# drowe67/pirip

Hardware: AMD Instinct MI355X
Metric: IQ Msamples/s demodulated (2-FSK Fs=240k Rs=10k); BER vs CPU ref (higher is better)
Workload: dtype f32

## Files before the change

pirip_amd/csrc/demod_simd.hpp:

```cpp
#pragma once
#include <hip/hip_runtime.h>

#include <cstdint>

#include "../../include/pirip_hip.h"

namespace pirip {

typedef float v2f __attribute__((ext_vector_type(2)));

__device__ __forceinline__ uint32_t fbits(float v) { return __builtin_bit_cast(uint32_t, v); }

__device__ __forceinline__ void wave_lds_sync()
{
    __builtin_amdgcn_fence(__ATOMIC_RELEASE, "wavefront");
    __builtin_amdgcn_wave_barrier();
    asm volatile("" ::: "memory");
    __builtin_amdgcn_fence(__ATOMIC_ACQUIRE, "wavefront");
}

#define PIRIP_DPP_F(old, src, ctrl, rmask) \
    __builtin_bit_cast(float, __builtin_amdgcn_update_dpp(__builtin_bit_cast(int, (float)(old)), __builtin_bit_cast(int, (float)(src)), ctrl, rmask, 0xf, false))

__device__ __forceinline__ float wave_sum(float v)
{
    v += PIRIP_DPP_F(0.f, v, 0x111, 0xf);
    v += PIRIP_DPP_F(0.f, v, 0x112, 0xf);
    v += PIRIP_DPP_F(0.f, v, 0x114, 0xf);
    v += PIRIP_DPP_F(0.f, v, 0x118, 0xf);
    v += PIRIP_DPP_F(0.f, v, 0x142, 0xa);
    v += PIRIP_DPP_F(0.f, v, 0x143, 0xc);
    return __builtin_bit_cast(float, __builtin_amdgcn_readlane(__builtin_bit_cast(int, v), 63));
}

#define PIRIP_DPP_REDUCE(op) \
        "s_nop 1\n\t" op " %0, %0, %0 row_shr:1 row_mask:0xf bank_mask:0xf\n\t" \
        "s_nop 1\n\t" op " %0, %0, %0 row_shr:2 row_mask:0xf bank_mask:0xf\n\t" \
        "s_nop 1\n\t" op " %0, %0, %0 row_shr:4 row_mask:0xf bank_mask:0xf\n\t" \
        "s_nop 1\n\t" op " %0, %0, %0 row_shr:8 row_mask:0xf bank_mask:0xf\n\t" \
        "s_nop 1\n\t" op " %0, %0, %0 row_bcast:15 row_mask:0xa bank_mask:0xf\n\t" \
        "s_nop 1\n\t" op " %0, %0, %0 row_bcast:31 row_mask:0xc bank_mask:0xf\n\t" \
        "s_nop 1\n\tv_readlane_b32 %1, %0, 63"

__device__ __forceinline__ void wave_argmax(float &v, int &idx)
{
    float red = v;
    int smax, smin;
    asm(PIRIP_DPP_REDUCE("v_max_f32_dpp") : "+v"(red), "=s"(smax));
    int cand = (__builtin_bit_cast(int, v) == smax) ? idx : 0x7fffffff;
    asm(PIRIP_DPP_REDUCE("v_min_i32_dpp") : "+v"(cand), "=s"(smin));
    v = __builtin_bit_cast(float, smax);
    idx = smin;
}

template <bool FINITE, bool NZ = false>
__device__ __forceinline__ float sqrt_rn_normal(float x)
{
    if (FINITE) {
        float q = __builtin_amdgcn_rsqf(x);
        if (!NZ) asm("v_min_f32 %0, %0, %1" : "+v"(q) : "v"(0x1p60f));
        const float y = x * q, h = 0.5f * q;
        return __builtin_fmaf(__builtin_fmaf(-y, y, x), h, y);
    }
    const float y = __builtin_amdgcn_sqrtf(x);
    const float ym = __builtin_bit_cast(float, __builtin_bit_cast(int, y) - 1);
    const float yp = __builtin_bit_cast(float, __builtin_bit_cast(int, y) + 1);
    const float rm = __builtin_fmaf(-ym, y, x);
    const float rp = __builtin_fmaf(-yp, y, x);
    float r = (rm <= 0.0f) ? ym : y;
    r = (rp > 0.0f) ? yp : r;
    return r;
}

__device__ __forceinline__ v2f cmul_x(v2f a, v2f t)
{
    v2f p2, r;
    asm("v_pk_mul_f32 %0, %2, %3 op_sel_hi:[0,1]\n\t"
        "v_pk_mul_f32 %1, %2, %3 op_sel:[1,1] op_sel_hi:[1,0]\n\t"
        "v_pk_add_f32 %0, %0, %1 neg_lo:[0,1]"
        : "=&v"(r), "=&v"(p2) : "v"(a), "v"(t));
    return r;
}
// ... 54 lines not shown
```

pirip_amd/csrc/fsk_demod_wave.hip:

```cpp
#include <hip/hip_runtime.h>

#include <cmath>
#include <cstdio>
#include <cstdlib>

#include "../../include/pirip_hip.h"
#include "demod_simd.hpp"
#include "fsk_device.hpp"

namespace pirip {

namespace {

constexpr int kWave = 64;

struct cf { float x, y; };

__device__ __forceinline__ float add_lane_up(float a, float b)
{
    float r;
    asm("v_add_f32_dpp %0, %1, %2 wave_shl:1 row_mask:0xf bank_mask:0xf bound_ctrl:0" : "=v"(r) : "v"(a), "v"(b));
    return r;
}

// ... 20 lines not shown
constexpr unsigned kQuickHi = 0x7c000000u;
__device__ __forceinline__ unsigned umin2(unsigned a, unsigned b) { return a < b ? a : b; }
__device__ __forceinline__ unsigned umin3(unsigned a, unsigned b, unsigned c)
{
    unsigned r;
    asm("v_min3_u32 %0, %1, %2, %3" : "=v"(r) : "v"(a), "v"(b), "v"(c));
    return r;
}

__device__ __forceinline__ v2f scale_lo(v2f h, v2f x)
{
    v2f r; asm("v_pk_mul_f32 %0, %1, %2 op_sel_hi:[0,1]" : "=v"(r) : "v"(h), "v"(x)); return r;
}
__device__ __forceinline__ v2f scale_hi(v2f h, v2f x)
{
    v2f r; asm("v_pk_mul_f32 %0, %1, %2 op_sel:[1,0] op_sel_hi:[1,1]" : "=v"(r) : "v"(h), "v"(x)); return r;
}
__device__ __forceinline__ float mag2(v2f w)
{
    v2f sq;
    asm("v_pk_mul_f32 %0, %1, %1" : "=v"(sq) : "v"(w));
    float r;
    asm("v_add_f32 %0, %1, %2" : "=v"(r) : "v"(sq.x), "v"(sq.y));
    return r;
}
__device__ __forceinline__ v2f smooth2(v2f sf, v2f mag, v2f k)
{
    v2f t;
    asm("v_pk_mul_f32 %0, %0, %3 op_sel_hi:[1,0]\n\t"
        "v_pk_mul_f32 %1, %2, %3 op_sel:[0,1] op_sel_hi:[1,1]\n\t"
        "v_pk_add_f32 %0, %0, %1"
        : "+v"(sf), "=&v"(t) : "v"(mag), "v"(k));
    return sf;
}

template <int FMT> struct InFmt;
template <> struct InFmt<PIRIP_IN_CU8_FSKDEMOD> { static constexpr int BPS = 2; static constexpr bool NEUTRAL_OK = true; static constexpr uint32_t NEUTRAL = 0x7F7F7F7Fu; };
template <> struct InFmt<PIRIP_IN_CU8_CSDR> { static constexpr int BPS = 2; static constexpr bool NEUTRAL_OK = false; static constexpr uint32_t NEUTRAL = 0x80808080u; };
template <> struct InFmt<PIRIP_IN_CS16> { static constexpr int BPS = 4; static constexpr bool NEUTRAL_OK = true; static constexpr uint32_t NEUTRAL = 0u; };
template <> struct InFmt<PIRIP_IN_CF32> { static constexpr int BPS = 8; static constexpr bool NEUTRAL_OK = true; static constexpr uint32_t NEUTRAL = 0u; };

__device__ __forceinline__ float cvt_s16(float x)
{
    const float hi = x * 0.00133514404296875f;
    return __builtin_fmaf(x, -0x1.e60f04p-20f, hi);
}
template <int FMT>
__device__ __forceinline__ v2f decode(const uint32_t *rw, int k)
{
    if (FMT == PIRIP_IN_CU8_FSKDEMOD || FMT == PIRIP_IN_CU8_CSDR) {
        const uint32_t v = rw[k >> 1];
        return cvt_u8_pair<FMT>(v2f{(k & 1) ? ubyte2(v) : ubyte0(v), (k & 1) ? ubyte3(v) : ubyte1(v)});
    } else if (FMT == PIRIP_IN_CS16) {
        const uint32_t v = rw[k];
        return v2f{cvt_s16((float)(short)(v & 0xffffu)), cvt_s16((float)((int)v >> 16))};
    } else {
        return v2f{__builtin_bit_cast(float, rw[2 * k]), __builtin_bit_cast(float, rw[2 * k + 1])};
    }
}
template <int FMT>
__device__ __forceinline__ v2f lds_sample(const unsigned char *p)
{
    if (FMT == PIRIP_IN_CU8_FSKDEMOD || FMT == PIRIP_IN_CU8_CSDR) {
        const uint32_t v = *(const uint16_t *)p;
        return cvt_u8_pair<FMT>(v2f{ubyte0(v), ubyte1(v)});
    } else if (FMT == PIRIP_IN_CS16) {
// ... 58 lines not shown
    static constexpr int NMEM = N + 2 * TS;
    static constexpr int Q = TS / 4;
    static constexpr int HIST = 2 * TS + Q;
    static constexpr int STEP = TS / P;
    static constexpr int NLANES = NSYM + 2;
    static constexpr int NFFT = (N - Q) / (NDFT / 2) - 1;
    static constexpr int GUARD_B = ((HIST * BPS + 15) / 16) * 16;
    static constexpr int SUP_B = (N + Q) * BPS;
    static constexpr int NDMA16 = SUP_B / 1024;
    static constexpr int NDMA4 = (SUP_B - NDMA16 * 1024 + 255) / 256;
    static constexpr bool DIRECT = FMT == PIRIP_IN_CF32 && NDFT >= 256;
    static constexpr int HEAD_B = 1024, DUMP_B = 256;
    static_assert(!DIRECT || ((TS + Q) * BPS <= HEAD_B && 3 * TS >= 2 * TS + Q), "the head holds blocks 0..2's new samples");
    static constexpr int RAW_B = DIRECT ? GUARD_B + HEAD_B + DUMP_B : GUARD_B + NDMA16 * 1024 + NDMA4 * 256;
    static constexpr int XPS256 = 16 * 17 * 8;
    static constexpr int XP_FFT_B = NDFT == 256 ? 4 * XPS256 : NDFT == 512 ? 4480 : 8 * 72 * 8;
    static constexpr int XP_B = cmax(cmax(XP_FFT_B, NDFT * 4), NDFT == 256 ? 64 * 20 * 4 : NDFT == 128 ? 8 * 136 * 4 : 0);
    static constexpr int TAIL_DW = HIST * BPS / 4;
    static constexpr int TRAILER_DW = GUARD_B / 4;
    static_assert((HIST * BPS) % 4 == 0 && (GUARD_B - HIST * BPS) % 4 == 0, "tail copies move whole dwords");
    static_assert(GUARD_B + (2 * M + 1) * 4 <= M * HIST * 8, "the state block holds the raw tail and its trailer");
    static constexpr int CHS = (BPS == 2) ? TS : (TS % 8 == 0 ? 8 : TS % 4 == 0 ? 4 : 2);
    static constexpr int CH_DW = CHS * BPS / 4;
    static_assert(TS % 2 == 0 && TS % P == 0 && P >= 4, "bad Ts / P");
    static_assert(NLANES <= kWave, "one lane per symbol block");
    static_assert((TS * BPS) % 16 == 0 && (CHS * BPS) % 16 == 0 && TS % CHS == 0, "block and chunk strides keep 16-byte alignment");
    static_assert((N + Q) / (NDFT / 2) - 1 == NFFT && N / (NDFT / 2) - 1 == NFFT, "numffts must not depend on nin");
    static_assert(NDFT == 256 ? (NFFT >= 4) : NDFT == 512 ? (NFFT % 2 == 0) : (NDFT == 128 && NFFT <= 8),
                  "FFT batches (Ndft = 256: the last batch of 4 may be partial; Ndft = 128: one batch of up to eight)");
    static_assert((NFFT - 1) * (NDFT / 2) + NDFT <= N - Q, "FFT windows stay inside the shortest frame");
    static_assert(M * P <= 48, "window prefix sums are kept in registers");
};

template <class C, int M> constexpr int wave_lds_bytes() { return C::RAW_B + C::XP_B; }

}

template <int M, int TS, int P, int NSYM, int NDFT, int FMT, int WPB, int WPS, bool FFT_FMA = false, bool MASK = false, int BAND = 0>
__global__ __launch_bounds__(kWave * WPB, WPS) void fsk_demod_wave_kernel(DemodArgs a_kernarg, int nstreams)
{
    constexpr bool INPLACE = TS == 10;
    static_assert(offsetof(DemodArgs, d) == 0, "the argument block is the first kernel argument");
    auto ap = [&]() {
        if constexpr (INPLACE) return (const __attribute__((address_space(4))) DemodArgs *)__builtin_amdgcn_kernarg_segment_ptr();
        else return (const DemodArgs *)&a_kernarg;
    }();
#define PIRIP_ARGS_REREAD() do { if constexpr (INPLACE) asm volatile("" : "+s"(ap)); } while (0)
#define a (*ap)
#define d (ap->d)
    static_assert(BAND == 0 || ((BAND == 2 || BAND == 4) && NDFT == 256 && !MASK), "band-only estimator: Ndft = 256, peak method, 32 or 64 bins");
    auto cmul = [](v2f x, v2f t) { return FFT_FMA ? rot_step(x, t) : cmul_x(x, t); };
    using C = WaveCfg<M, TS, P, NSYM, NDFT, FMT>;
    constexpr int N = C::N, NMEM = C::NMEM, HIST = C::HIST, STEP = C::STEP, Q = C::Q, BPS = C::BPS;
    constexpr int GUARD_B = C::GUARD_B;

    __shared__ __attribute__((aligned(16))) unsigned char s_raw[WPB][C::RAW_B];
    __shared__ __attribute__((aligned(16))) unsigned char s_xp[WPB][C::XP_B];
    constexpr int TAB_F = NDFT == 256 ? 12 * 16 * 4 : NDFT == 512 ? 8 * 16 * 2 + 12 * 32 * 2 : 8 * 16 * 2;
    __shared__ __attribute__((aligned(16))) float s_tab[TAB_F];
    __shared__ __attribute__((aligned(16))) float2 s_tph[P];
    __shared__ __attribute__((aligned(16))) float2 s_tgain[NSYM + 2];
    __shared__ float s_misc[WPB][3];
    extern __shared__ __attribute__((aligned(16))) float s_lnI0[];

    const int lane0 = threadIdx.x & (kWave - 1);
    const int wv = __builtin_amdgcn_readfirstlane(threadIdx.x >> 6);
    const int sid = blockIdx.x * WPB + wv;

    if (NDFT == 256) {
        for (int i = threadIdx.x; i < 12 * 16; i += kWave * WPB)
            ((float4 *)s_tab)[i] = ((const float4 *)a.t.fast_tab)[(i & 15) * 12 + (i >> 4)];
    } else {
        for (int i = threadIdx.x; i < TAB_F / 4; i += kWave * WPB) ((float4 *)s_tab)[i] = ((const float4 *)(a.t.fast_tab + NDFT))[i];
    }
    if constexpr (P <= 10) if (a.io.soft.llr) {
        if (a.io.soft.llr_map == kLlrRician) { for (int i = threadIdx.x; i < 258; i += kWave * WPB) s_lnI0[i] = a.io.soft.lnI0[i]; }
        else if (threadIdx.x < 20) {
            const int sg = threadIdx.x >> 2, cc = threadIdx.x & 3;
            const float c2 = sg == 0 ? 0.226f : sg == 1 ? 0.1245f : sg == 2 ? 0.0288f : sg == 3 ? 0.002f : 0.0f;
            const float c1 = sg == 0 ? 0.0125f : sg == 1 ? 0.2177f : sg == 2 ? 0.6314f : sg == 3 ? 0.9048f : 0.9867f;
            const float c0 = sg == 0 ? -0.0012f : sg == 1 ? -0.108f : sg == 2 ? -0.5645f : sg == 3 ? -1.2997f : -2.2053f;
            s_lnI0[threadIdx.x] = cc == 0 ? c2 : cc == 1 ? c1 : cc == 2 ? c0 : 0.0f;
        }
    }
    if (threadIdx.x < P) s_tph[threadIdx.x] = a.t.tph[threadIdx.x];
    if (threadIdx.x < NSYM + 2) s_tgain[threadIdx.x] = a.t.timing_rec[(threadIdx.x < NSYM + 1 ? threadIdx.x : 0) * P];
    __syncthreads();
    if (sid >= nstreams) return;
    if (a.io.seg && a.io.seg[sid].max_frames < 0) return;

    unsigned char *raw = s_raw[wv];
    unsigned char *xpb = s_xp[wv];

    uint32_t *st32 = (uint32_t *)(a.s.hist + (size_t)sid * M * HIST);
    int ninp = __builtin_amdgcn_readfirstlane((int)st32[C::TRAILER_DW + 2 * M]);
    uint32_t dthp[M];
    int tixp[M];
#pragma unroll
    for (int m = 0; m < M; m++) {
        dthp[m] = (uint32_t)__builtin_amdgcn_readfirstlane((int)st32[C::TRAILER_DW + m]);
        tixp[m] = __builtin_amdgcn_readfirstlane((int)st32[C::TRAILER_DW + M + m]);
    }
    for (int i = lane0; i < GUARD_B / 4; i += kWave) ((uint32_t *)raw)[i] = ninp ? st32[i] : InFmt<FMT>::NEUTRAL;

#define PIRIP_PHASE_LANE(name) int name = lane0; asm volatile("" : "+v"(name))
    constexpr int NOWN = NDFT / kWave;
    constexpr int NB = BAND ? BAND : NOWN;
    auto own_sfi = [](int ln, int b) {
        const int bin = BAND ? ((ln & 15) + 16 * b)
                      : NDFT == 256 ? ((ln & 15) + 16 * b + 64 * (ln >> 4)) : NDFT == 512 ? ((ln & 31) + 32 * (8 * (ln >> 5) + b)) : (ln + 64 * b);
        return (bin + NDFT / 2) & (NDFT - 1);
    };
    float Sf[NOWN];
    float hann16[NDFT == 256 ? 1 : 16];
    if constexpr (NDFT == 512) {
#pragma unroll
        for (int i = 0; i < 16; i++) hann16[i] = a.t.fast_tab[(lane0 & 31) + 32 * (i >> 3) + 64 * (i & 7)];
    }
    if constexpr (NDFT == 128) {
#pragma unroll
        for (int i = 0; i < 16; i++) hann16[i] = a.t.fast_tab[(lane0 & 7) + 8 * i];
    }
#pragma unroll
    for (int b = 0; b < NB; b++) Sf[b] = a.s.Sf[(size_t)sid * NDFT + own_sfi(lane0, b)];

    float sc_norm_rx_timing, sc_ppm, sc_SNRest;
    int sc_nin;
    {
        const StreamScalars sc = a.s.scal[sid];
        sc_norm_rx_timing = sc.norm_rx_timing; sc_ppm = sc.ppm; sc_SNRest = sc.SNRest; sc_nin = sc.nin;
        if (lane0 == 0) { s_misc[wv][0] = sc.snr_est; s_misc[wv][1] = sc.EbNodB; s_misc[wv][2] = sc.v_est; }
    }

    int64_t seg_in = 0, out0 = 0, max_frames = a.io.max_frames;
    if (a.io.seg) {
        const SegDesc sd = a.io.seg[sid];
        seg_in = sd.in_off; out0 = sd.out_frame0; max_frames = sd.max_frames;
    }
    const uint8_t *in_base = a.io.in + (size_t)sid * a.io.in_stride + (size_t)seg_in * BPS;
    const int64_t nsamp = a.io.nsamp - seg_in;
    const __amdgpu_buffer_rsrc_t rsrc =
        __builtin_amdgcn_make_buffer_rsrc((void *)in_base, 0, (int)(uint32_t)(BPS * nsamp), 0x00020000);

    int nin = __builtin_amdgcn_readfirstlane(sc_nin);
    int64_t pos = 0, frame = 0;
    if (a.io.first) { pos = __builtin_amdgcn_readfirstlane(a.io.first[sid]); frame = pos ? 1 : 0; }
    const int64_t frame_first = frame;
    int last_freqi0 = 0, last_freqi1 = 0, last_freqi2 = 0, last_freqi3 = 0;

    typedef __attribute__((address_space(3))) void *lds_ptr;
    auto dma_frame = [&](int64_t p0) {
        const uint32_t goff = (uint32_t)__builtin_amdgcn_readfirstlane((int)(uint32_t)(p0 * BPS));
        if constexpr (C::DIRECT) {
            __builtin_amdgcn_raw_ptr_buffer_load_lds(rsrc, (lds_ptr)(raw + GUARD_B), 16, lane0 * 16, goff, 0, 0);
#pragma unroll
            for (int i = 0; i < (C::SUP_B + 8191) / 8192; i++)
                __builtin_amdgcn_raw_ptr_buffer_load_lds(rsrc, (lds_ptr)(raw + GUARD_B + C::HEAD_B), 4, lane0 * 128, goff + i * 8192, 0, 0);
            return;
        }
#pragma unroll
        for (int i = 0; i < C::NDMA16; i++)
            __builtin_amdgcn_raw_ptr_buffer_load_lds(rsrc, (lds_ptr)(raw + GUARD_B + i * 1024), 16, lane0 * 16, goff + i * 1024, 0, 0);
#pragma unroll
        for (int i = 0; i < C::NDMA4; i++)
            __builtin_amdgcn_raw_ptr_buffer_load_lds(rsrc, (lds_ptr)(raw + GUARD_B + C::NDMA16 * 1024 + i * 256), 4, lane0 * 4,
                                                     goff + C::NDMA16 * 1024 + i * 256, 0, 0);
    };
    constexpr bool SOFT_OK = P <= 10;
    uint32_t soft_carry = 0;
    int soft_cb = 0, soft_w = 0;
    uint32_t *words_o = nullptr;
    if constexpr (SOFT_OK) if (a.io.soft.llr) { words_o = a.io.soft.words + (size_t)sid * a.io.soft.words_stride + (a.io.soft.bit0 >> 5); }
    auto soft_append = [&](uint32_t W, int nb) {
        const uint32_t merged = soft_carry | (soft_cb ? (W >> soft_cb) : W);
        if (soft_cb + nb >= 32) {
            if (lane0 == 0) words_o[soft_w] = merged;
            soft_w++;
            soft_carry = soft_cb ? (W << (32 - soft_cb)) : 0u;
            soft_cb = soft_cb + nb - 32;
        } else { soft_carry = merged; soft_cb += nb; }
    };
// ... 395 lines not shown
#pragma unroll
                        for (int u = 0; u < 8; u++) { A[u] = sqrtf(A[u]); B[u] = sqrtf(B[u]); __builtin_amdgcn_sched_barrier(0); }
                    }
                }
#pragma unroll
                for (int u = 0; u < 8; u += 2) {
                    v2f sp{Sf[u], Sf[u + 1]};
                    sp = smooth2(sp, v2f{A[u], A[u + 1]}, ktc);
                    sp = smooth2(sp, v2f{B[u], B[u + 1]}, ktc);
                    Sf[u] = sp.x; Sf[u + 1] = sp.y;
                }
                wave_lds_sync();
            }
        }

        __builtin_amdgcn_sched_barrier(0);
        PIRIP_T_MARK(1);
        int freqi[M];
#pragma unroll
        for (int m = 0; m < M; m++) freqi[m] = 0;
        int bb = 0;
        if constexpr (MASK) {
            PIRIP_PHASE_LANE(lane);
            float *sfl = (float *)xpb;
#pragma unroll
            for (int b = 0; b < NOWN; b++) sfl[own_sfi(lane, b)] = Sf[b];
            wave_lds_sync();
            float best = 0.0f; int ib = d.est_st;
            for (int b = d.est_st + lane; b < d.est_en - d.mask_len; b += kWave) {
                float corr = 0.0f;
                for (int k = 0; k < d.n_teeth; k++) corr += sfl[b + a.t.teeth[k]];
                if (corr > best) { best = corr; ib = b; }
            }
            wave_argmax(best, ib);
            bb = ib;
            wave_lds_sync();
        } else {
            PIRIP_PHASE_LANE(lane);
            float w[NB];
            int sfi[NB];
#pragma unroll
            for (int b = 0; b < NB; b++) {
                sfi[b] = (BAND && lane >= 16) ? -1 : own_sfi(lane, b);
                w[b] = (sfi[b] >= d.est_st && sfi[b] < d.est_en) ? Sf[b] : 0.0f;
            }
#pragma unroll
            for (int m = 0; m < M; m++) {
                float best = 0.0f; int ib = 0;
#pragma unroll
                for (int b = 0; b < NB; b++)
                    if (w[b] > best) { best = w[b]; ib = sfi[b]; }
                wave_argmax(best, ib);
                int f_min = ib - d.f_zero; f_min = f_min < 0 ? 0 : f_min;
                int f_max = ib + d.f_zero; f_max = f_max > NDFT ? NDFT : f_max;
#pragma unroll
                for (int b = 0; b < NB; b++) if (sfi[b] >= f_min && sfi[b] < f_max) w[b] = 0.0f;
                freqi[m] = ib - NDFT / 2;
            }
#pragma unroll
            for (int x = 1; x < M; x++)
#pragma unroll
                for (int y = x; y > 0; y--)
                    if (freqi[y] < freqi[y - 1]) { const int t = freqi[y]; freqi[y] = freqi[y - 1]; freqi[y - 1] = t; }
        }
        constexpr int LOG2N = NDFT == 128 ? 7 : NDFT == 256 ? 8 : 9;
        uint32_t dthv[M];
        int tix[M];
#pragma unroll
        for (int m = 0; m < M; m++) {
            if constexpr (MASK) { dthv[m] = a.t.mask_dtheta[bb * M + m]; tix[m] = bb * M + m; }
            else { dthv[m] = (uint32_t)freqi[m] << (32 - LOG2N); tix[m] = freqi[m] + NDFT / 2; }
        }

        auto phasor = [&](uint32_t th) {
            const float2 w = a.t.tw[th >> (32 - LOG2N)];
            float pc = w.x, ps = -w.y;
            if constexpr (MASK) {
                const float bl = (float)(th & ((1u << (32 - LOG2N)) - 1u)) * 1.4629180792671596e-9f;
                const float b2 = bl * bl;
                const float cb = 1.0f - b2 * (0.5f - b2 * (1.0f / 24.0f));
                const float sb = bl * (1.0f - b2 * ((1.0f / 6.0f) - b2 * (1.0f / 120.0f)));
                const float c2 = pc * cb - ps * sb, s2 = ps * cb + pc * sb;
                pc = c2; ps = s2;
            }
            return make_float2(pc, ps);
        };
        __builtin_amdgcn_sched_barrier(0);
        PIRIP_T_MARK(2);
        v2f fi[M][P];
        v2f tot[M];
        {
            PIRIP_PHASE_LANE(lane);
            const int lb = lane < C::NLANES ? lane : C::NLANES - 1;
            const int boff = GUARD_B + (TS * lb - nold) * BPS;
            const int al = (GUARD_B - nold * BPS) & 15;
            v2f ph[M], dph[M], acc[M];
            v2f sw_ph[M], sw_dph[M];
            const int n0 = TS * lb - nold + 1;
            const int nold_blk = nold - TS * lb;
            const bool oldl = nold_blk > 0;
#pragma unroll
            for (int m = 0; m < M; m++) {
                const float2 stn = a.t.osc_step[tix[m]], stp = a.t.osc_step[tixp[m]];
                const float dn = a.t.osc_drift[tix[m]].x, dp = a.t.osc_drift[tixp[m]].x;
                const uint32_t th = (uint32_t)n0 * (oldl ? dthp[m] : dthv[m]);
                const float g = 1.0f + (oldl ? dp * (float)(ninp + n0) : dn * (float)n0);
                const float2 pcs = phasor(th);
                ph[m] = v2f{pcs.x * g, pcs.y * g};
                dph[m] = oldl ? v2f{stp.x, stp.y} : v2f{stn.x, stn.y};
                const float2 p1 = phasor(dthv[m]);
                const float g1 = 1.0f + dn;
                sw_ph[m] = v2f{p1.x * g1, p1.y * g1};
                sw_dph[m] = v2f{stn.x, stn.y};
                acc[m] = v2f{0.f, 0.f};
            }
            const int zero_blk = ninp ? 0 : nold_blk;
#pragma unroll
            for (int c = 0; c < TS / C::CHS; c++) {
                uint32_t rw[C::CH_DW];
                if (C::DIRECT && lb >= 3) {
#pragma unroll
                    for (int i = 0; i < C::CH_DW / 4; i++) {
                        const auto v = __builtin_amdgcn_raw_buffer_load_b128(rsrc, (TS * lb - nold) * BPS + c * C::CHS * BPS + 16 * i, (int)goff_frame, 0);
                        const uint4 u = __builtin_bit_cast(uint4, v);
                        rw[4 * i] = u.x; rw[4 * i + 1] = u.y; rw[4 * i + 2] = u.z; rw[4 * i + 3] = u.w;
                    }
                } else {
                    const unsigned char *bp = raw + boff + c * C::CHS * BPS;
                    if (al == 0) {
#pragma unroll
                        for (int i = 0; i < C::CH_DW / 4; i++) {
                            const uint4 v = ((const uint4 *)bp)[i];
                            rw[4 * i] = v.x; rw[4 * i + 1] = v.y; rw[4 * i + 2] = v.z; rw[4 * i + 3] = v.w;
                        }
                    } else if ((al & 7) == 0) {
#pragma unroll
                        for (int i = 0; i < C::CH_DW / 2; i++) { const uint2 v = ((const uint2 *)bp)[i]; rw[2 * i] = v.x; rw[2 * i + 1] = v.y; }
                    } else {
#pragma unroll
                        for (int i = 0; i < C::CH_DW; i++) rw[i] = ((const uint32_t *)bp)[i];
                    }
                }
#pragma unroll
                for (int kk = 0; kk < C::CHS; kk++) {
                    const int k = c * C::CHS + kk;
                    {
                        uint32_t &v0 = rw[BPS == 2 ? (kk >> 1) : (BPS == 4 ? kk : 2 * kk)];
                        if (M == 2) asm volatile("" : "+v"(v0), "+v"(ph[0]), "+v"(ph[M - 1]));
                        else asm volatile("" : "+v"(v0), "+v"(ph[0]), "+v"(ph[1]), "+v"(ph[M - 2]), "+v"(ph[M - 1]));
// ... 19 lines not shown
#pragma unroll
                    for (int m = 0; m < M; m++) {
                        if (k % STEP == 0) fi[m][k / STEP] = acc[m];
                        acc[m] = nacc[m];
                    }
                    if ((kk & 3) == 3) __builtin_amdgcn_sched_barrier(0);
                }
            }
#pragma unroll
            for (int m = 0; m < M; m++) tot[m] = acc[m];
        }
        PIRIP_PHASE_LANE(lane);
        if constexpr (C::DIRECT) {
            asm volatile("s_waitcnt lgkmcnt(0)" ::: "memory");
            wave_lds_sync();
            const uint32_t toff = (uint32_t)__builtin_amdgcn_readfirstlane((int)(uint32_t)((pos + nin - HIST) * BPS));
#pragma unroll
            for (int i = 0; i < (C::TAIL_DW + kWave - 1) / kWave; i++)
                if (lane + i * kWave < C::TAIL_DW)
                    __builtin_amdgcn_raw_ptr_buffer_load_lds(rsrc, (lds_ptr)(raw + GUARD_B - HIST * BPS + i * 256), 4, lane * 4, toff + i * 256, 0, 0);
        } else {
            const uint32_t *tsrc = (const uint32_t *)(raw + GUARD_B + (nin - HIST) * BPS);
            uint32_t *tdst = (uint32_t *)(raw + GUARD_B - HIST * BPS);
            uint32_t tv[(C::TAIL_DW + kWave - 1) / kWave];
#pragma unroll
            for (int i = 0; i < (C::TAIL_DW + kWave - 1) / kWave; i++) tv[i] = tsrc[lane + i * kWave < C::TAIL_DW ? lane + i * kWave : 0];
#pragma unroll
            for (int i = 0; i < (C::TAIL_DW + kWave - 1) / kWave; i++) if (lane + i * kWave < C::TAIL_DW) tdst[lane + i * kWave] = tv[i];
        }
        asm volatile("s_waitcnt lgkmcnt(0)" ::: "memory");
        wave_lds_sync();
        PIRIP_T_MARK(3);
        dma_frame(pos + nin);
        ninp = nin;
#pragma unroll
        for (int m = 0; m < M; m++) { dthp[m] = dthv[m]; tixp[m] = tix[m]; }

        float tcr = 0.f, tci = 0.f;
        {
            v2f prpi{0.f, 0.f};
            v2f ft{0.f, 0.f};
#pragma unroll
            for (int q = 0; q < P; q++) {
#pragma unroll
                for (int m = 0; m < M; m++) {
                    const v2f own = fi[m][q];
                    v2f w0;
                    w0.x = add_lane_up(own.x, tot[m].x - own.x);
                    w0.y = add_lane_up(own.y, tot[m].y - own.y);
                    fi[m][q] = w0;
                    if (m == 0) asm("v_mul_f32 %0, %1, %1\n\tv_fma_f32 %0, %2, %2, %0" : "=&v"(ft.x) : "v"(w0.y), "v"(w0.x));
                    else { float t2; asm("v_mul_f32 %0, %2, %2\n\tv_fma_f32 %0, %3, %3, %0\n\tv_add_f32 %1, %1, %0" : "=&v"(t2), "+v"(ft.x) : "v"(w0.y), "v"(w0.x)); }
                }
                const v2f tp = *(const v2f *)&s_tph[q];
                asm("v_pk_fma_f32 %0, %1, %2, %0 op_sel_hi:[0,1,1]" : "+v"(prpi) : "v"(ft), "v"(tp));
                asm volatile("" : "+v"(prpi), "+v"(fi[0][q]), "+v"(fi[M - 1][q]));
            }
            const float pr = prpi.x, pi = prpi.y;
            if (lane <= NSYM) {
                const float2 tgain = s_tgain[lane];
                tcr = pr * tgain.x - pi * tgain.y;
                tci = pr * tgain.y + pi * tgain.x;
            }
            tcr = wave_sum(tcr); tci = wave_sum(tci);
        }

        PIRIP_T_MARK(4);
        PIRIP_ARGS_REREAD();
        const int frame_bytes = d.pack_bits ? (d.Nbits + 7) / 8 : d.Nbits;
        const size_t orow = (size_t)(frame + out0);
        uint8_t *bits_o = a.io.bits ? a.io.bits + (size_t)sid * a.io.bits_stride + orow * frame_bytes : nullptr;
        float *filt_o = a.io.filt ? a.io.filt + (size_t)sid * a.io.filt_stride + orow * M * NSYM : nullptr;
        float *stats_o = a.io.stats ? a.io.stats + (size_t)sid * a.io.stats_stride + orow * PIRIP_STATS_PER_FRAME : nullptr;
        float f_est[kMaxTones] = {0.f, 0.f, 0.f, 0.f};
#pragma unroll
        for (int m = 0; m < M; m++) {
            if constexpr (MASK) f_est[m] = (float)((bb - NDFT / 2) * d.Fs / NDFT) + (float)(m * d.tone_spacing);
            else f_est[m] = (float)freqi[m] * d.bin_hz;
        }

        const bool bad = isnan(tcr) || isnan(tci);
        int nin_next = nin;
        if (!bad) {
            const float norm_rx_timing = FMT == PIRIP_IN_CF32 ? atan2f(tci, tcr) * 0.15915494309189535f : atan2_turns(tci, tcr);
            const float rx_timing = norm_rx_timing * (float)P;
            const float d_norm = norm_rx_timing - sc_norm_rx_timing;
            sc_norm_rx_timing = norm_rx_timing;
            if (fabsf(d_norm) < 0.2f) {
                const float appm = (1e6f * d_norm) / (float)NSYM;
                sc_ppm = (0.9f * sc_ppm) + (0.1f * appm);
            }
            nin_next = N;
            if (!d.burst_mode) {
                if (norm_rx_timing > 0.25f) nin_next = N + Q;
                else if (norm_rx_timing < -0.25f) nin_next = N - Q;
            }

            const int low_sample = __builtin_amdgcn_readfirstlane((int)floorf(rx_timing));
            const float fract = rx_timing - (float)low_sample;
            const int high_sample = __builtin_amdgcn_readfirstlane((int)ceilf(rx_timing));
            v2f lo[M], hi[M];
            {
                const int ql = low_sample >= 0 ? low_sample : P + low_sample;
                const int qh = high_sample >= 0 ? high_sample : P + high_sample;
#define PIRIP_SEL_CASE(q) case q: if (q < P) { asm volatile(""); for (int m_ = 0; m_ < M; m_++) DST[m_] = fi[m_][q < P ? q : 0]; } break;
#define PIRIP_SELECT(idx) do { switch (idx) { \
    PIRIP_SEL_CASE(0) PIRIP_SEL_CASE(1) PIRIP_SEL_CASE(2) PIRIP_SEL_CASE(3) PIRIP_SEL_CASE(4) PIRIP_SEL_CASE(5) \
    PIRIP_SEL_CASE(6) PIRIP_SEL_CASE(7) PIRIP_SEL_CASE(8) PIRIP_SEL_CASE(9) PIRIP_SEL_CASE(10) PIRIP_SEL_CASE(11) \
    PIRIP_SEL_CASE(12) PIRIP_SEL_CASE(13) PIRIP_SEL_CASE(14) PIRIP_SEL_CASE(15) PIRIP_SEL_CASE(16) PIRIP_SEL_CASE(17) \
    PIRIP_SEL_CASE(18) PIRIP_SEL_CASE(19) PIRIP_SEL_CASE(20) PIRIP_SEL_CASE(21) PIRIP_SEL_CASE(22) PIRIP_SEL_CASE(23) \
    default: break; } } while (0)
                static_assert(P <= 24, "selection switch covers 24 window starts");
#pragma unroll
// ... 115 lines not shown
            }
            const bool last_frame = (frame + 1 >= max_frames) || (pos + nin + nin_next > nsamp);
            if (stats_o || last_frame) {
                float sig = act ? mx : 0.f, nse = act ? (sum - mx) / (float)(M - 1) : 0.f;
                sig = wave_sum(sig); nse = wave_sum(nse) + 1e-12f;
                sig = sig / (float)NSYM; nse = nse / (float)NSYM;
                sc_SNRest = sig / nse;
                float mean_e = wave_sum(act ? sqrtf(mx) : 0.f), std_e = wave_sum(act ? mx : 0.f);
                mean_e = mean_e / (float)NSYM;
                std_e = (std_e / (float)NSYM) - (mean_e * mean_e);
                std_e = std_e > 0.0f ? sqrtf(std_e) : 0.0f;
                const float EbNodB = -6.0f + (20.0f * log10f((1e-6f + mean_e) / (1e-6f + std_e)));
                if (lane == 0) {
                    s_misc[wv][0] = (0.5f * s_misc[wv][0]) + (0.5f * EbNodB);
                    s_misc[wv][1] = EbNodB;
                    s_misc[wv][2] = sqrtf(sig - nse);
                    a.s.scal[sid].rx_sig_pow = sig; a.s.scal[sid].rx_nse_pow = nse;
                    if (stats_o) { stats_o[8] = sig; stats_o[9] = nse; }
                }
            }
        } else {
            for (int i = lane; i < frame_bytes; i += kWave) if (bits_o) bits_o[i] = 0;
            for (int i = lane; i < M * NSYM; i += kWave) if (filt_o) filt_o[i] = 0.f;
            if (stats_o && lane == 0) { stats_o[8] = 0.f; stats_o[9] = 0.f; }
            if constexpr (SOFT_OK) if (a.io.soft.llr) {
                uint16_t *llr_o = a.io.soft.llr + (size_t)sid * a.io.soft.llr_stride + a.io.soft.bit0 + (size_t)frame * NBITS;
                for (int i = lane; i < NBITS; i += kWave) llr_o[i] = 0;
                for (int j = 0; j < (NBITS + 31) / 32; j++) soft_append(0u, (j + 1) * 32 <= NBITS ? 32 : NBITS - 32 * j);
            }
        }
        if constexpr (MASK) last_freqi0 = bb;
        else { last_freqi0 = freqi[0]; last_freqi1 = freqi[M > 1 ? 1 : 0]; last_freqi2 = freqi[M > 2 ? 2 : 0]; last_freqi3 = freqi[M > 3 ? 3 : 0]; }
        if (stats_o && lane == 0) {
            stats_o[0] = f_est[0]; stats_o[1] = f_est[1]; stats_o[2] = f_est[2]; stats_o[3] = f_est[3];
            stats_o[4] = sc_norm_rx_timing; stats_o[5] = sc_SNRest; stats_o[6] = (float)nin_next; stats_o[7] = sc_ppm;
        }
        PIRIP_T_MARK(5);
        pos += nin;
        nin = __builtin_amdgcn_readfirstlane(nin_next);
        frame++;
        wave_lds_sync();
    }

    if constexpr (SOFT_OK) if (words_o && soft_cb > 0 && lane0 == 0) words_o[soft_w] = soft_carry;
    asm volatile("s_waitcnt vmcnt(0)" ::: "memory");
#ifdef PIRIP_WAVE_TIMING
    if (a.io.stats && lane0 == 0 && sid == nstreams / 2)
        for (int i = 0; i < 8; i++) a.io.stats[(size_t)sid * a.io.stats_stride + i] = (float)t_acc_[i];
#endif
#pragma unroll
    for (int b = 0; b < NB; b++) if (!BAND || lane0 < 16) a.s.Sf[(size_t)sid * NDFT + own_sfi(lane0, b)] = Sf[b];
    wave_lds_sync();
    for (int i = lane0; i < GUARD_B / 4; i += kWave) st32[i] = ((const uint32_t *)raw)[i];
    const int lane = lane0;
    if (lane == 0) {
#pragma unroll
        for (int m = 0; m < M; m++) { st32[C::TRAILER_DW + m] = dthp[m]; st32[C::TRAILER_DW + M + m] = (uint32_t)tixp[m]; }
        st32[C::TRAILER_DW + 2 * M] = (uint32_t)ninp;
        StreamScalars sc = a.s.scal[sid];
        sc.nin = nin; sc.norm_rx_timing = sc_norm_rx_timing; sc.ppm = sc_ppm; sc.SNRest = sc_SNRest;
        sc.snr_est = s_misc[wv][0]; sc.EbNodB = s_misc[wv][1]; sc.v_est = s_misc[wv][2];
        if (frame > frame_first) {
            const int fq[4] = {last_freqi0, last_freqi1, last_freqi2, last_freqi3};
            for (int m = 0; m < kMaxTones; m++) {
                if (MASK) sc.f_est[m] = m < M ? (float)((fq[0] - NDFT / 2) * d.Fs / NDFT) + (float)(m * d.tone_spacing) : 0.f;
                else sc.f_est[m] = m < M ? (float)fq[m] * d.bin_hz : 0.f;
            }
        }
        a.s.scal[sid] = sc;
        if (a.io.nframes) a.io.nframes[sid] = (int32_t)frame;
        if (a.io.consumed) a.io.consumed[sid] = pos;
    }
#undef a
#undef d
#undef PIRIP_ARGS_REREAD
}

namespace {
__global__ void sqrt_selftest_kernel(unsigned long long *bad, unsigned lo, unsigned hi)
{
    unsigned long long c = 0;
    const unsigned stride = gridDim.x * blockDim.x;
    for (unsigned long long b = (unsigned long long)lo + blockIdx.x * blockDim.x + threadIdx.x; b <= hi; b += stride) {
        const float x = __builtin_bit_cast(float, (unsigned)b);
        const float want = (float)sqrt((double)x);
        if (__builtin_bit_cast(unsigned, sqrt_rn_normal<true>(x)) != __builtin_bit_cast(unsigned, want)) c++;
        if (x != 0.0f && __builtin_bit_cast(unsigned, sqrt_rn_normal<true, true>(x)) != __builtin_bit_cast(unsigned, want)) c++;
        if (__builtin_bit_cast(unsigned, sqrt_rn_normal<false>(x)) != __builtin_bit_cast(unsigned, want)) c += 1ull << 32;
    }
    if (c) atomicAdd(bad, c);
}
}

hipError_t selftest_sqrt(unsigned long long *mismatches)
{
// ... 147 lines not shown
```

pirip_amd/csrc/fsk_plan.cpp:

```cpp
#include "fsk_plan.hpp"

#include <cassert>
#include <cmath>
#include <cstdlib>
#include <cstring>
#include <string>

#include "../../include/pirip_hip.h"

namespace pirip {

namespace {
struct cf { float re, im; };
inline cf cmul(cf a, cf b) { return {a.re * b.re - a.im * b.im, a.re * b.im + a.im * b.re}; }
}

int FskPlan::init(int Fs, int Rs, int M, int P, int Nsym, int est_min, int est_max,
                  int freq_est_type, int tone_spacing, int in_format, const pirip_fsk_recalled *recalled)
{
    pirip_fsk_recalled rc;
    recalled_defaults(&rc);
    const pirip_fsk_recalled dflt = rc;
    if (recalled) rc = *recalled;
    if (!(rc.tc > 0.0f && rc.tc <= 1.0f) || !(rc.est_space_rs >= 0.0f) || !(rc.nin_threshold > 0.0f && rc.nin_threshold < 0.5f) || rc.nin_step_div < 2 ||
// ... 13 lines not shown
    int Ndft = (int)Ndft_f;
    if (rc.ndft_rule == 1) { Ndft = 1; while (2 * Ndft <= (Fs / Rs) * Nsym) Ndft *= 2; }
    if (Ndft < 8 || Ndft > 16384) return PIRIP_ERR_BAD_CONFIG;
    if ((Fs / Rs) / rc.nin_step_div < 1) return PIRIP_ERR_BAD_CONFIG;

    d.Fs = Fs; d.Rs = Rs; d.M = M; d.P = P; d.Nsym = Nsym;
    d.Ts = Fs / Rs;
    d.N = d.Ts * Nsym;
    d.Nmem = d.N + 2 * d.Ts;
    d.Ndft = Ndft;
    d.Nbits = (M == 2) ? Nsym : 2 * Nsym;
    d.nint = (Nsym + 1) * P;
    d.tc = rc.tc;
    d.one_minus_tc = 1 - d.tc;
    d.nin_step = d.Ts / rc.nin_step_div;
    d.nin_thresh = rc.nin_threshold;
    d.s16_scale = rc.s16_scale;
    d.sf_power = rc.sf_power;
    d.u8_table = (in_format == PIRIP_IN_CU8_FSKDEMOD && (rc.u8d_offset != dflt.u8d_offset || rc.u8d_scale != dflt.u8d_scale)) ? 1 : 0;
    d.recalled_fast_ok = (rc.nin_threshold == dflt.nin_threshold && rc.nin_step_div == dflt.nin_step_div && rc.s16_scale == dflt.s16_scale &&
                          !d.u8_table && rc.ndft_rule == dflt.ndft_rule && rc.sf_power == dflt.sf_power) ? 1 : 0;
    d.freq_est_type = freq_est_type ? 1 : 0;
    d.tone_spacing = tone_spacing;
    d.in_format = in_format;
    d.hist_len = 2 * d.Ts + d.nin_step;
    {
        const int step = d.Ts / P;
        auto gcd = [](int a, int b) { while (b) { const int t = a % b; a = b; b = t; } return a; };
        d.grp = gcd(gcd(step, d.nin_step > 0 ? d.nin_step : step), d.hist_len);
        if (d.grp < 1) d.grp = 1;
    }
    d.burst_mode = 0;
    d.block_stagger = 0;
    d.fft_fma = 0;
    d.est_band = 0;
    d.pack_bits = 0;
    d.bin_hz = (float)Fs / (float)Ndft;

    const int est_space = rc.est_space_rs * Rs;
    if (!fsk_est_range(Fs, Ndft, est_min, est_max, &d.est_st, &d.est_en)) return PIRIP_ERR_BAD_CONFIG;
    d.f_zero = (est_space * Ndft) / Fs;

    hann.resize(Ndft);
    {
        const float w = rc.hann_denominator_ndft ? (2 * M_PI) / ((float)Ndft) : (2 * M_PI) / ((float)Ndft - 1);
        cf dphi{cosf(w), sinf(w)};
        cf rphi{.5f, 0.0f};
        rphi = cmul(cf{dphi.re, -dphi.im}, rphi);
        for (int i = 0; i < Ndft; i++) {
            rphi = cmul(dphi, rphi);
            hann[i] = .5f - rphi.re;
        }
    }

    twiddle.resize(2 * (size_t)Ndft);
    for (int i = 0; i < Ndft; i++) {
        const double pi = 3.141592653589793238462643383279502884197169399375105820974944;
        double phase = -2 * pi * i / Ndft;
        twiddle[2 * i] = (float)std::cos(phase);
        twiddle[2 * i + 1] = (float)std::sin(phase);
    }

    int radices[kMaxStages], ms[kMaxStages], nst = 0;
    {
        int n = Ndft;
        while (n > 1) {
// ... 326 lines not shown
```

pirip_amd/csrc/fsk_plan.hpp:

```cpp
#pragma once
#include <cstdint>
#include <vector>

#include "../../include/pirip_hip.h"

namespace pirip {

constexpr int kMaxTones = 4;
constexpr int kMaxStages = 16;

struct FftStage { int radix; int m; int fstride; };

struct FskDims {
    int Fs, Rs, M, P, Nsym;
    int Ts, N, Nmem, Ndft, Nbits, nint;
    int est_st, est_en, f_zero;
    int freq_est_type;
    int tone_spacing;
    int mask_len;
    int n_teeth;
    int in_format;
    int hist_len;
    int grp;
    int nstages;
    int pack_bits;
    int burst_mode;
    int fft_fma;
    int est_band;
    float tc, one_minus_tc;
    float bin_hz;
    int nin_step;
    float nin_thresh;
    float s16_scale;
    int u8_table;
    int sf_power;
    int recalled_fast_ok;
    int block_stagger;
};

struct FskPlan {
    FskDims d{};
    FftStage stages[kMaxStages]{};
    std::vector<float> hann;
    std::vector<float> twiddle;
    std::vector<uint16_t> leaf_perm;
    std::vector<uint16_t> leaf_iperm;
    std::vector<float> u8_lut;
    std::vector<float> timing_ph;
    std::vector<int16_t> teeth;
    std::vector<uint32_t> mask_dtheta;
    std::vector<float> osc_drift;
    std::vector<float> osc_step;
    std::vector<float> timing_rec;
    std::vector<float> fast_tab;
    float tw_s2[18];
    int init(int Fs, int Rs, int M, int P, int Nsym, int est_min, int est_max,
             int freq_est_type, int tone_spacing, int in_format, const pirip_fsk_recalled *recalled = nullptr);
};

struct FskMod {
    int Fs, Rs, M, Ts, f1_tx, tone_spacing;
    float ph_re = 1.0f, ph_im = 0.0f;
    void init(int Fs_, int Rs_, int M_, int f1, int spacing);
    void mod(const uint8_t *bits, int nbits, float *out, bool complex_out);
};

void test_frame_bits(uint8_t *frame, int framesize);

struct PutBits {
    int framesize; float valid_thresh;
// ... 16 lines not shown
```

pirip_amd/csrc/pirip_capi.hip:

```cpp
#include <hip/hip_runtime.h>

#include <cstdio>
#include <cstdlib>
#include <cstring>
#include <new>
#include <vector>

#include "../../include/pirip_hip.h"
#include "fsk_device.hpp"
#include "fsk_plan.hpp"
#include "demod_handle.hpp"

using namespace pirip;

namespace {

int reset_state(pirip_hip_demod *h, hipStream_t st)
{
    const FskDims &d = h->plan.d;
    const size_t ns = (size_t)h->nstreams;
    PIRIP_HIPCHK(hipMemsetAsync(h->d_Sf, 0, sizeof(float) * ns * d.Ndft, st));
    PIRIP_HIPCHK(hipMemsetAsync(h->d_theta, 0, sizeof(uint32_t) * ns * kMaxTones, st));
    PIRIP_HIPCHK(hipMemsetAsync(h->d_hist, 0, sizeof(float2) * ns * d.M * d.hist_len, st));
    PIRIP_HIPCHK(hipMemsetAsync(h->d_phic, 0, sizeof(float2) * ns * kMaxTones, st));
// ... 128 lines not shown
    return pirip_hip_create_recalled(p, nullptr, nstreams, device, out);
}

int pirip_hip_create_recalled(const pirip_fsk_params *p, const pirip_fsk_recalled *recalled, int nstreams, int device, pirip_hip_demod **out)
{
    if (!p || !out || nstreams <= 0) return PIRIP_ERR_BAD_ARG;
    *out = nullptr;
    pirip_hip_demod *h = new (std::nothrow) pirip_hip_demod();
    if (!h) return PIRIP_ERR_NOMEM;
    pirip_fsk_recalled from_env;
    if (!recalled && getenv("PIRIP_RECALLED")) {
        recalled_defaults(&from_env);
        if (!recalled_from_env(&from_env)) { delete h; return PIRIP_ERR_BAD_CONFIG; }
        recalled = &from_env;
    }
    int rc = h->plan.init(p->Fs, p->Rs, p->M, p->P, p->Nsym, p->est_min, p->est_max,
                          p->freq_est_type, p->tone_spacing, p->in_format, recalled);
    if (rc != PIRIP_OK) { delete h; return rc; }
    if (demod_general_lds_bytes(h->plan.d) > 160 * 1024) { delete h; return PIRIP_ERR_UNSUPPORTED; }

    rc = select_device(device, &h->device);
    if (rc != PIRIP_OK) { delete h; return rc; }
    h->nstreams = nstreams;
    {
        const char *k = getenv("PIRIP_KERNEL");
        const bool want_general = getenv("PIRIP_FORCE_GENERAL") || (k && !strcmp(k, "general"));
        if (const char *f = getenv("PIRIP_FFT_FMA")) {
            h->plan.d.fft_fma = atoi(f) ? 1 : 0;
            if (h->plan.d.fft_fma && !demod_wave_applicable(h->plan.d)) h->plan.d.fft_fma = 0;
        }
        h->kernel = want_general || !h->plan.d.recalled_fast_ok ? 0 :
                    demod_wave_applicable(h->plan.d) ? PIRIP_KERNEL_WAVE : demod_block_applicable(h->plan.d) ? PIRIP_KERNEL_BLOCK : 0;
        if (const char *sg = getenv("PIRIP_BLOCK_STAGGER")) h->plan.d.block_stagger = atoi(sg) > 0 ? atoi(sg) : 0;
        if (const char *b = getenv("PIRIP_EST_BAND")) {
            if (atoi(b)) h->plan.d.est_band = est_band_for(h);
        }
        if (k && !strcmp(k, "exact")) {
            h->plan.d.grp = 1;
            if (!demod_exact_applicable(h->plan.d)) { delete h; return PIRIP_ERR_UNSUPPORTED; }
            h->kernel = PIRIP_KERNEL_EXACT;
        }
    }

    rc = alloc_tables_and_state(h);
    if (rc != PIRIP_OK) { delete h; return rc; }
    if (const char *e = getenv("PIRIP_EXACT0")) h->exact0 = atoi(e) ? 1 : 0;
    rc = reset_state(h, nullptr);
    if (rc != PIRIP_OK) { delete h; return rc; }
    *out = h;
    return PIRIP_OK;
}

int pirip_hip_destroy(pirip_hip_demod *h)
{
    if (!h) return PIRIP_ERR_BAD_ARG;
    (void)bind(h);
    (void)hipDeviceSynchronize();
    pirip::capture_release(h);
    delete h;
    return PIRIP_OK;
}

int pirip_hip_get_kernel(const pirip_hip_demod *h) { return h ? h->kernel : PIRIP_ERR_BAD_ARG; }

int pirip_hip_get_kernel_name(const pirip_hip_demod *h, char *buf, size_t n)
{
// ... 333 lines not shown
```

Before: 350,400.

## Cache oscillator phasors across frames and add single-holder argmax shortcut

Adds a per-wave frame cache for the oscillator starting phasors and steps. Frames whose nin, previous nin and tone indices are unchanged reuse the cached values instead of recomputing phasors and reloading step and drift tables. The argmax gains a ballot fast path that skips the second DPP min-reduction when one lane holds the maximum, and the est-range test becomes a precomputed bitmask AND. The f_est computation moves into the stats branch. Instance-selection tables choose per template configuration which paths are enabled, at the cost of more register state and branch complexity.

```diff
diff --git a/pirip_amd/csrc/demod_simd.hpp b/pirip_amd/csrc/demod_simd.hpp
--- a/pirip_amd/csrc/demod_simd.hpp
+++ b/pirip_amd/csrc/demod_simd.hpp
@@ -42,12 +42,22 @@
         "s_nop 1\n\t" op " %0, %0, %0 row_bcast:31 row_mask:0xc bank_mask:0xf\n\t" \
         "s_nop 1\n\tv_readlane_b32 %1, %0, 63"
 
+template <bool SINGLE = false>
 __device__ __forceinline__ void wave_argmax(float &v, int &idx)
 {
     float red = v;
     int smax, smin;
     asm(PIRIP_DPP_REDUCE("v_max_f32_dpp") : "+v"(red), "=s"(smax));
-    int cand = (__builtin_bit_cast(int, v) == smax) ? idx : 0x7fffffff;
+    const bool holds = __builtin_bit_cast(int, v) == smax;
+    if constexpr (SINGLE) {
+        const unsigned long long who = __ballot(holds);
+        if (__builtin_popcountll(who) == 1) {
+            v = __builtin_bit_cast(float, smax);
+            idx = __builtin_amdgcn_readlane(idx, __builtin_ctzll(who));
+            return;
+        }
+    }
+    int cand = holds ? idx : 0x7fffffff;
     asm(PIRIP_DPP_REDUCE("v_min_i32_dpp") : "+v"(cand), "=s"(smin));
     v = __builtin_bit_cast(float, smax);
     idx = smin;
diff --git a/pirip_amd/csrc/fsk_demod_wave.hip b/pirip_amd/csrc/fsk_demod_wave.hip
--- a/pirip_amd/csrc/fsk_demod_wave.hip
+++ b/pirip_amd/csrc/fsk_demod_wave.hip
@@ -76,6 +76,22 @@
         "v_pk_add_f32 %0, %0, %1"
         : "+v"(sf), "=&v"(t) : "v"(mag), "v"(k));
     return sf;
+}
+
+template <int B>
+__device__ __forceinline__ uint32_t flag_mask_at(uint32_t flags)
+{
+    uint32_t r;
+    asm("v_bfe_i32 %0, %1, %2, 1" : "=v"(r) : "v"(flags), "n"(B));
+    return r;
+}
+__device__ __forceinline__ uint32_t flag_mask(uint32_t flags, int b)
+{
+    switch (b) {
+    case 0: return flag_mask_at<0>(flags); case 1: return flag_mask_at<1>(flags); case 2: return flag_mask_at<2>(flags);
+    case 3: return flag_mask_at<3>(flags); case 4: return flag_mask_at<4>(flags); case 5: return flag_mask_at<5>(flags);
+    case 6: return flag_mask_at<6>(flags); default: return flag_mask_at<7>(flags);
+    }
 }
 
 template <int FMT> struct InFmt;
@@ -200,6 +216,21 @@
     static_assert(M * P <= 48, "window prefix sums are kept in registers");
 };
 
+constexpr bool wave_plain_instance(int M, int TS, int P, int NDFT, int FMT, int WPS, bool FFT_FMA, bool MASK, int BAND)
+{
+    if (MASK && M == 4) return true;
+    if (MASK && M == 2 && TS == 24 && FMT == PIRIP_IN_CU8_CSDR) return true;
+    if (!MASK && M == 4 && FMT == PIRIP_IN_CF32 && (TS == 18 || TS == 10)) return true;
+    return false;
+}
+
+constexpr bool wave_two_pass_argmax_instance(int M, int TS, int FMT, bool MASK, int BAND)
+{
+    if (MASK && M == 2 && TS == 24) return true;
+    if (!MASK && M == 4 && (FMT == PIRIP_IN_CF32 || FMT == PIRIP_IN_CS16 || BAND == 4)) return true;
+    return false;
+}
+
 template <class C, int M> constexpr int wave_lds_bytes() { return C::RAW_B + C::XP_B; }
 
 }
@@ -208,6 +239,8 @@
 __global__ __launch_bounds__(kWave * WPB, WPS) void fsk_demod_wave_kernel(DemodArgs a_kernarg, int nstreams)
 {
     constexpr bool INPLACE = TS == 10;
+    constexpr bool PLAIN = wave_plain_instance(M, TS, P, NDFT, FMT, WPS, FFT_FMA, MASK, BAND);
+    constexpr bool ARGMAX_SINGLE = !PLAIN && !wave_two_pass_argmax_instance(M, TS, FMT, MASK, BAND);
     static_assert(offsetof(DemodArgs, d) == 0, "the argument block is the first kernel argument");
     auto ap = [&]() {
         if constexpr (INPLACE) return (const __attribute__((address_space(4))) DemodArgs *)__builtin_amdgcn_kernarg_segment_ptr();
@@ -261,7 +294,7 @@
     unsigned char *xpb = s_xp[wv];
 
     uint32_t *st32 = (uint32_t *)(a.s.hist + (size_t)sid * M * HIST);
-    int ninp = __builtin_amdgcn_readfirstlane((int)st32[C::TRAILER_DW + 2 * M]);
+    const int ninp0 = __builtin_amdgcn_readfirstlane((int)st32[C::TRAILER_DW + 2 * M]);
     uint32_t dthp[M];
     int tixp[M];
 #pragma unroll
@@ -269,7 +302,7 @@
         dthp[m] = (uint32_t)__builtin_amdgcn_readfirstlane((int)st32[C::TRAILER_DW + m]);
         tixp[m] = __builtin_amdgcn_readfirstlane((int)st32[C::TRAILER_DW + M + m]);
     }
-    for (int i = lane0; i < GUARD_B / 4; i += kWave) ((uint32_t *)raw)[i] = ninp ? st32[i] : InFmt<FMT>::NEUTRAL;
+    for (int i = lane0; i < GUARD_B / 4; i += kWave) ((uint32_t *)raw)[i] = ninp0 ? st32[i] : InFmt<FMT>::NEUTRAL;
 
 #define PIRIP_PHASE_LANE(name) int name = lane0; asm volatile("" : "+v"(name))
     constexpr int NOWN = NDFT / kWave;
@@ -315,6 +348,29 @@
     if (a.io.first) { pos = __builtin_amdgcn_readfirstlane(a.io.first[sid]); frame = pos ? 1 : 0; }
     const int64_t frame_first = frame;
     int last_freqi0 = 0, last_freqi1 = 0, last_freqi2 = 0, last_freqi3 = 0;
+
+    uint32_t in_range = 0;
+    if constexpr (!MASK && !PLAIN) {
+#pragma unroll
+        for (int b = 0; b < NB; b++) {
+            const int sfi = (BAND && lane0 >= 16) ? -1 : own_sfi(lane0, b);
+            if (sfi >= d.est_st && sfi < d.est_en) in_range |= 1u << b;
+        }
+    }
+    constexpr bool FCACHE = WPS <= 3 && !PLAIN;
+    constexpr bool KEEP_STEP = FCACHE && (M == 2 || WPS == 2);
+    constexpr uint32_t kFcStale = 0x40000000u, kFcNever = 0x80000000u, kFcRan = 0x20000000u;
+    static_assert(N + Q < 0x10000, "last frame's length leaves the flag bits free");
+    v2f ph_c[FCACHE ? M : 1], step_c[KEEP_STEP ? M : 1];
+    if constexpr (FCACHE) {
+#pragma unroll
+        for (int m = 0; m < M; m++) ph_c[m] = v2f{0.f, 0.f};
+    }
+    if constexpr (KEEP_STEP) {
+#pragma unroll
+        for (int m = 0; m < M; m++) step_c[m] = v2f{0.f, 0.f};
+    }
+    uint32_t ninp_fc = (uint32_t)ninp0 | (d.frame_cache ? kFcStale : kFcNever);
 
     typedef __attribute__((address_space(3))) void *lds_ptr;
     auto dma_frame = [&](int64_t p0) {
@@ -776,17 +832,19 @@
                 for (int k = 0; k < d.n_teeth; k++) corr += sfl[b + a.t.teeth[k]];
                 if (corr > best) { best = corr; ib = b; }
             }
-            wave_argmax(best, ib);
+            wave_argmax<ARGMAX_SINGLE>(best, ib);
             bb = ib;
             wave_lds_sync();
         } else {
             PIRIP_PHASE_LANE(lane);
             float w[NB];
             int sfi[NB];
+            static_assert(NB <= 8, "one flag bit per owned bin");
 #pragma unroll
             for (int b = 0; b < NB; b++) {
                 sfi[b] = (BAND && lane >= 16) ? -1 : own_sfi(lane, b);
-                w[b] = (sfi[b] >= d.est_st && sfi[b] < d.est_en) ? Sf[b] : 0.0f;
+                if constexpr (PLAIN) w[b] = (sfi[b] >= d.est_st && sfi[b] < d.est_en) ? Sf[b] : 0.0f;
+                else w[b] = __builtin_bit_cast(float, fbits(Sf[b]) & flag_mask(in_range, b));
             }
 #pragma unroll
             for (int m = 0; m < M; m++) {
@@ -794,7 +852,7 @@
 #pragma unroll
                 for (int b = 0; b < NB; b++)
                     if (w[b] > best) { best = w[b]; ib = sfi[b]; }
-                wave_argmax(best, ib);
+                wave_argmax<ARGMAX_SINGLE>(best, ib);
                 int f_min = ib - d.f_zero; f_min = f_min < 0 ? 0 : f_min;
                 int f_max = ib + d.f_zero; f_max = f_max > NDFT ? NDFT : f_max;
 #pragma unroll
@@ -843,22 +901,46 @@
             const int n0 = TS * lb - nold + 1;
             const int nold_blk = nold - TS * lb;
             const bool oldl = nold_blk > 0;
-#pragma unroll
-            for (int m = 0; m < M; m++) {
-                const float2 stn = a.t.osc_step[tix[m]], stp = a.t.osc_step[tixp[m]];
-                const float dn = a.t.osc_drift[tix[m]].x, dp = a.t.osc_drift[tixp[m]].x;
-                const uint32_t th = (uint32_t)n0 * (oldl ? dthp[m] : dthv[m]);
-                const float g = 1.0f + (oldl ? dp * (float)(ninp + n0) : dn * (float)n0);
-                const float2 pcs = phasor(th);
-                ph[m] = v2f{pcs.x * g, pcs.y * g};
-                dph[m] = oldl ? v2f{stp.x, stp.y} : v2f{stn.x, stn.y};
-                const float2 p1 = phasor(dthv[m]);
-                const float g1 = 1.0f + dn;
-                sw_ph[m] = v2f{p1.x * g1, p1.y * g1};
-                sw_dph[m] = v2f{stn.x, stn.y};
-                acc[m] = v2f{0.f, 0.f};
-            }
+            const int ninp = (int)(ninp_fc & 0xffffu);
             const int zero_blk = ninp ? 0 : nold_blk;
+            uint32_t moved = (uint32_t)(nin ^ N) | (uint32_t)(ninp ^ N);
+#pragma unroll
+            for (int m = 0; m < M; m++) moved |= (uint32_t)(tix[m] ^ tixp[m]);
+            static_assert(Q > 0 && Q < TS, "a block changes oscillators at sample Ts/4 or Ts - Ts/4 only: never where nold_blk is a multiple of Ts");
+            if (FCACHE && (moved | (ninp_fc & (kFcStale | kFcNever))) == 0) {
+#pragma unroll
+                for (int m = 0; m < M; m++) {
+                    if constexpr (KEEP_STEP) dph[m] = step_c[m];
+                    else { const float2 stn = a.t.osc_step[tix[m]]; dph[m] = v2f{stn.x, stn.y}; }
+                    if constexpr (FCACHE) ph[m] = ph_c[m];
+                    sw_ph[m] = dph[m];
+                    sw_dph[m] = dph[m];
+                }
+            } else {
+#pragma unroll
+                for (int m = 0; m < M; m++) {
+                    const float2 stn = a.t.osc_step[tix[m]], stp = a.t.osc_step[tixp[m]];
+                    const float dn = a.t.osc_drift[tix[m]].x, dp = a.t.osc_drift[tixp[m]].x;
+                    const uint32_t th = (uint32_t)n0 * (oldl ? dthp[m] : dthv[m]);
+                    const float g = 1.0f + (oldl ? dp * (float)(ninp + n0) : dn * (float)n0);
+                    const float2 pcs = phasor(th);
+                    ph[m] = v2f{pcs.x * g, pcs.y * g};
+                    dph[m] = oldl ? v2f{stp.x, stp.y} : v2f{stn.x, stn.y};
+                    const float2 p1 = phasor(dthv[m]);
+                    const float g1 = 1.0f + dn;
+                    sw_ph[m] = v2f{p1.x * g1, p1.y * g1};
+                    sw_dph[m] = v2f{stn.x, stn.y};
+                    if constexpr (FCACHE) ph_c[m] = ph[m];
+                    if constexpr (KEEP_STEP) step_c[m] = sw_dph[m];
+                }
+            }
+            if constexpr (KEEP_STEP) {
+#pragma unroll
+                for (int m = 0; m < M; m++) sw_dph[m] = step_c[m];
+            }
+            ninp_fc = (uint32_t)nin | (PLAIN ? 0u : kFcRan) | (ninp_fc & kFcNever) | (FCACHE ? ((moved + (kFcStale - 1u)) & kFcStale) : 0u);
+#pragma unroll
+            for (int m = 0; m < M; m++) acc[m] = v2f{0.f, 0.f};
 #pragma unroll
             for (int c = 0; c < TS / C::CHS; c++) {
                 uint32_t rw[C::CH_DW];
@@ -944,7 +1026,6 @@
         wave_lds_sync();
         PIRIP_T_MARK(3);
         dma_frame(pos + nin);
-        ninp = nin;
 #pragma unroll
         for (int m = 0; m < M; m++) { dthp[m] = dthv[m]; tixp[m] = tix[m]; }
 
@@ -979,18 +1060,11 @@
 
         PIRIP_T_MARK(4);
         PIRIP_ARGS_REREAD();
-        const int frame_bytes = d.pack_bits ? (d.Nbits + 7) / 8 : d.Nbits;
+        const int frame_bytes = d.pack_bits ? (NBITS + 7) / 8 : NBITS;
         const size_t orow = (size_t)(frame + out0);
         uint8_t *bits_o = a.io.bits ? a.io.bits + (size_t)sid * a.io.bits_stride + orow * frame_bytes : nullptr;
         float *filt_o = a.io.filt ? a.io.filt + (size_t)sid * a.io.filt_stride + orow * M * NSYM : nullptr;
         float *stats_o = a.io.stats ? a.io.stats + (size_t)sid * a.io.stats_stride + orow * PIRIP_STATS_PER_FRAME : nullptr;
-        float f_est[kMaxTones] = {0.f, 0.f, 0.f, 0.f};
-#pragma unroll
-        for (int m = 0; m < M; m++) {
-            if constexpr (MASK) f_est[m] = (float)((bb - NDFT / 2) * d.Fs / NDFT) + (float)(m * d.tone_spacing);
-            else f_est[m] = (float)freqi[m] * d.bin_hz;
-        }
-
         const bool bad = isnan(tcr) || isnan(tci);
         int nin_next = nin;
         if (!bad) {
@@ -1172,6 +1246,12 @@
         if constexpr (MASK) last_freqi0 = bb;
         else { last_freqi0 = freqi[0]; last_freqi1 = freqi[M > 1 ? 1 : 0]; last_freqi2 = freqi[M > 2 ? 2 : 0]; last_freqi3 = freqi[M > 3 ? 3 : 0]; }
         if (stats_o && lane == 0) {
+            float f_est[kMaxTones] = {0.f, 0.f, 0.f, 0.f};
+#pragma unroll
+            for (int m = 0; m < M; m++) {
+                if constexpr (MASK) f_est[m] = (float)((bb - NDFT / 2) * d.Fs / NDFT) + (float)(m * d.tone_spacing);
+                else f_est[m] = (float)freqi[m] * d.bin_hz;
+            }
             stats_o[0] = f_est[0]; stats_o[1] = f_est[1]; stats_o[2] = f_est[2]; stats_o[3] = f_est[3];
             stats_o[4] = sc_norm_rx_timing; stats_o[5] = sc_SNRest; stats_o[6] = (float)nin_next; stats_o[7] = sc_ppm;
         }
@@ -1196,11 +1276,11 @@
     if (lane == 0) {
 #pragma unroll
         for (int m = 0; m < M; m++) { st32[C::TRAILER_DW + m] = dthp[m]; st32[C::TRAILER_DW + M + m] = (uint32_t)tixp[m]; }
-        st32[C::TRAILER_DW + 2 * M] = (uint32_t)ninp;
+        st32[C::TRAILER_DW + 2 * M] = ninp_fc & 0xffffu;
         StreamScalars sc = a.s.scal[sid];
         sc.nin = nin; sc.norm_rx_timing = sc_norm_rx_timing; sc.ppm = sc_ppm; sc.SNRest = sc_SNRest;
         sc.snr_est = s_misc[wv][0]; sc.EbNodB = s_misc[wv][1]; sc.v_est = s_misc[wv][2];
-        if (frame > frame_first) {
+        if (PLAIN ? frame > frame_first : (ninp_fc & kFcRan) != 0) {
             const int fq[4] = {last_freqi0, last_freqi1, last_freqi2, last_freqi3};
             for (int m = 0; m < kMaxTones; m++) {
                 if (MASK) sc.f_est[m] = m < M ? (float)((fq[0] - NDFT / 2) * d.Fs / NDFT) + (float)(m * d.tone_spacing) : 0.f;
diff --git a/pirip_amd/csrc/fsk_plan.cpp b/pirip_amd/csrc/fsk_plan.cpp
--- a/pirip_amd/csrc/fsk_plan.cpp
+++ b/pirip_amd/csrc/fsk_plan.cpp
@@ -69,6 +69,7 @@
     }
     d.burst_mode = 0;
     d.block_stagger = 0;
+    d.frame_cache = 1;
     d.fft_fma = 0;
     d.est_band = 0;
     d.pack_bits = 0;
diff --git a/pirip_amd/csrc/fsk_plan.hpp b/pirip_amd/csrc/fsk_plan.hpp
--- a/pirip_amd/csrc/fsk_plan.hpp
+++ b/pirip_amd/csrc/fsk_plan.hpp
@@ -36,6 +36,7 @@
     int sf_power;
     int recalled_fast_ok;
     int block_stagger;
+    int frame_cache;
 };
 
 struct FskPlan {
diff --git a/pirip_amd/csrc/pirip_capi.hip b/pirip_amd/csrc/pirip_capi.hip
--- a/pirip_amd/csrc/pirip_capi.hip
+++ b/pirip_amd/csrc/pirip_capi.hip
@@ -184,6 +184,7 @@
         h->kernel = want_general || !h->plan.d.recalled_fast_ok ? 0 :
                     demod_wave_applicable(h->plan.d) ? PIRIP_KERNEL_WAVE : demod_block_applicable(h->plan.d) ? PIRIP_KERNEL_BLOCK : 0;
         if (const char *sg = getenv("PIRIP_BLOCK_STAGGER")) h->plan.d.block_stagger = atoi(sg) > 0 ? atoi(sg) : 0;
+        if (const char *fc = getenv("PIRIP_FRAME_CACHE")) h->plan.d.frame_cache = atoi(fc) ? 1 : 0;
         if (const char *b = getenv("PIRIP_EST_BAND")) {
             if (atoi(b)) h->plan.d.est_band = est_band_for(h);
         }
```

Measured after the change: 361,200 (median of 6 runs). +3.1%, better.
